# UWQuickstep/quickstep

Measured on AMD Instinct MI355X. Metric: probe+aggregate rows/s at TPC-H SF100 (Q1,Q3), higher is better.
Workload: dtype i32 keys / f64 sums

## Files before the change

### quickstep_amd/csrc/aggregate.hip

```cpp

#include "agg_common.hpp"
#include "agg_translate.hpp"
#include "agg_hash_update.hpp"
#include "agg_factored.hpp"
#include "agg_shapes.hpp"
#include "agg_family.hpp"
#include "agg_pieces.hpp"
#include "agg_jit.hpp"
#include "comm.hpp"
#include "partition.hpp"
#include "scan.hpp"

#include <atomic>
#include <cstdlib>
#include <map>
#include <mutex>
#include <shared_mutex>
#include <vector>

namespace qsx {

struct ColKinds {
  int kind[QSX_MAX_AGGS + 1];
};

__global__ __launch_bounds__(kABlock) void fill_identity_kernel(unsigned long long *__restrict__ states, long long col_stride,
                                                               long long col_words, int num_cols, ColKinds kinds) {
  for (int col = 0; col < num_cols; ++col) {
    if (kinds.kind[col] < kAccMinI64) continue;
    const unsigned long long identity = static_cast<unsigned long long>(acc_identity(kinds.kind[col]));
    unsigned long long *p = states + static_cast<long long>(col) * col_stride;
    for (long long i = static_cast<long long>(blockIdx.x) * kABlock + threadIdx.x; i < col_words;
         i += static_cast<long long>(gridDim.x) * kABlock) {
      p[i] = identity;
    }
  }
}

__global__ __launch_bounds__(kABlock) void merge_hash_kernel(const unsigned long long *__restrict__ image,
                                                            unsigned long long src_cap, int num_cols,
                                                            ColKinds kinds, HashTableView g) {
  const unsigned long long *src_keys = image;
  const unsigned long long *src_states = image + (src_cap + 1);
  for (unsigned long long i = static_cast<unsigned long long>(blockIdx.x) * kABlock + threadIdx.x;
       i <= src_cap; i += static_cast<unsigned long long>(gridDim.x) * kABlock) {
    const unsigned long long cnt = src_states[i];
    if (cnt == 0) continue;
    const unsigned long long code = i == src_cap ? kEmptyCode : src_keys[i];
    if (i != src_cap && code == kEmptyCode) continue;
    const unsigned long long gs = global_find_or_insert(g, code);
    if (gs == ~0ull) continue;
    for (int col = 0; col < num_cols; ++col) {
      global_add(g, col, gs, src_states[static_cast<unsigned long long>(col) * (src_cap + 1) + i], kinds.kind[col]);
    }
  }
}

__global__ __launch_bounds__(kABlock) void merge_dense_kernel(const unsigned long long *__restrict__ image,
                                                             unsigned long long *__restrict__ dst,
                                                             long long exist_words, long long num_entries,
                                                             int num_cols, ColKinds kinds) {
  const long long total = exist_words + static_cast<long long>(num_cols) * num_entries;
  for (long long i = static_cast<long long>(blockIdx.x) * kABlock + threadIdx.x; i < total;
       i += static_cast<long long>(gridDim.x) * kABlock) {
    const unsigned long long v = image[i];
    if (i < exist_words) {
      if (v != 0) atomicOr(&dst[i], v);
    } else {
      const int kind = kinds.kind[static_cast<int>((i - exist_words) / num_entries)];
      if (v == static_cast<unsigned long long>(acc_identity(kind))) continue;
      global_accumulate(&dst[i], v, kind);
    }
  }
}

__global__ __launch_bounds__(kABlock) void init_log_kernel(unsigned long long *__restrict__ log, int stride,
                                                          unsigned long long count, const unsigned int *__restrict__ count_dev,
                                                          unsigned int log_cap, ColKinds kinds) {
  if (count_dev != nullptr) count = *count_dev < log_cap ? *count_dev : log_cap;
  const unsigned long long words = count * stride;
  for (unsigned long long i = static_cast<unsigned long long>(blockIdx.x) * kABlock + threadIdx.x; i < words;
       i += static_cast<unsigned long long>(gridDim.x) * kABlock) {
    const int w = static_cast<int>(i % stride);
    log[i] = w == 0 ? kEmptyCode : static_cast<unsigned long long>(acc_identity(kinds.kind[w - 1]));
  }
}

__global__ __launch_bounds__(kABlock) void drain_log_kernel(const unsigned long long *__restrict__ records, unsigned int count,
                                                           int stride, int num_cols, ColKinds kinds, HashTableView g) {
  for (unsigned int r = blockIdx.x * kABlock + threadIdx.x; r < count; r += gridDim.x * kABlock) {
    const unsigned long long *rec = records + static_cast<unsigned long long>(r) * stride;
    const unsigned long long gs = global_find_or_insert(g, rec[0]);
    if (gs == ~0ull) continue;
    for (int col = 0; col < num_cols; ++col) global_add(g, col, gs, rec[1 + col], kinds.kind[col]);
  }
}

__global__ void publish_control_kernel(const unsigned long long *__restrict__ control, unsigned long long *host_slot,
                                       unsigned long long seq) {
  if (threadIdx.x != 0) return;
  __hip_atomic_store(&host_slot[0], control[0], __ATOMIC_RELAXED, __HIP_MEMORY_SCOPE_SYSTEM);
  __hip_atomic_store(&host_slot[1], control[3], __ATOMIC_RELAXED, __HIP_MEMORY_SCOPE_SYSTEM);
  __hip_atomic_store(&host_slot[2], control[1], __ATOMIC_RELAXED, __HIP_MEMORY_SCOPE_SYSTEM);
  __hip_atomic_store(&host_slot[3], seq, __ATOMIC_RELEASE, __HIP_MEMORY_SCOPE_SYSTEM);
}


__device__ __forceinline__ double avg_quotient(double s, double c) {
  const double q = s / c;
  if (!isfinite(q) || fabs(q) >= 2.2250738585072014e-308) return q;
  double best = q, best_r = fabs(fma(-q, c, s));
  const double around[2] = {nextafter(q, -INFINITY), nextafter(q, INFINITY)};
  for (const double x : around) {
    const double r = fabs(fma(-x, c, s));
    if (r < best_r || (r == best_r && (__double_as_longlong(x) & 1) == 0)) {
      best = x;
      best_r = r;
    }
  }
  return best;
}

__device__ __forceinline__ void write_values(const FinalizeDesc &f, const unsigned long long *states,
                                             unsigned long long col_stride, unsigned long long idx,
                                             int count_col, bool empty_group, long long out_row) {
  const long long cnt = count_col >= 0 ? static_cast<long long>(states[static_cast<unsigned long long>(count_col) * col_stride + idx]) : 0;
  for (int a = 0; a < f.num_aggs; ++a) {
    bool is_null = false;
    const bool has_nn = f.nn_col[a] >= 0;
    const long long seen = has_nn ? static_cast<long long>(states[static_cast<unsigned long long>(f.nn_col[a]) * col_stride + idx]) : cnt;
    if (f.fn[a] == QSX_AGG_COUNT_STAR) {
      static_cast<long long *>(f.out_vals[a])[out_row] = cnt;
    } else if (f.fn[a] == QSX_AGG_COUNT) {
      static_cast<long long *>(f.out_vals[a])[out_row] = seen;
    } else {
      const unsigned long long raw = states[static_cast<unsigned long long>(f.sum_col[a]) * col_stride + idx];
      if (f.fn[a] == QSX_AGG_SUM) {
        is_null = empty_group || (has_nn && seen == 0);
        static_cast<unsigned long long *>(f.out_vals[a])[out_row] = is_null ? 0ull : raw;
      } else if (f.fn[a] == QSX_AGG_MIN || f.fn[a] == QSX_AGG_MAX) {
        is_null = empty_group || (has_nn ? seen == 0 : (count_col >= 0 && cnt == 0));
        const long long word = static_cast<long long>(raw);
        switch (f.val_type[a]) {
          case QSX_INT: static_cast<int32_t *>(f.out_vals[a])[out_row] = is_null ? 0 : static_cast<int32_t>(word); break;
          case QSX_LONG: static_cast<long long *>(f.out_vals[a])[out_row] = is_null ? 0 : word; break;
          case QSX_FLOAT:
            static_cast<float *>(f.out_vals[a])[out_row] = is_null ? 0.0f : static_cast<float>(__longlong_as_double(ordered_from_bits(word)));
            break;
          default:
            static_cast<double *>(f.out_vals[a])[out_row] = is_null ? 0.0 : __longlong_as_double(ordered_from_bits(word));
            break;
        }
      } else {
        const double sum = f.is_int[a] ? static_cast<double>(static_cast<long long>(raw))
                                       : __longlong_as_double(static_cast<long long>(raw));
        is_null = seen == 0;
        static_cast<double *>(f.out_vals[a])[out_row] = is_null ? 0.0 : avg_quotient(sum, static_cast<double>(seen));
      }
// ... 739 lines not shown
}
static int dir_plane_sums(const DevConfig &dev) { return dev.num_sums - 2 * dev.wide_words; }
static size_t dir_lds_bytes(int tile_bytes, int temps_bytes, int num_sums, int gids, int nbuf) {
  return static_cast<size_t>(nbuf) * tile_bytes + temps_bytes + static_cast<size_t>(gids + kWave) * (8 * static_cast<size_t>(num_sums) + 4) + 16;
}

struct DenseLdsGeometry {
  int entries;
  int rep_shift;
  int ranges;
};
static DenseLdsGeometry dense_lds_geometry(long long num_entries, int num_sums, size_t tile_and_temps_bytes, bool allow_families) {
  const char *e = getenv("QSX_AGG_DENSE_LDS");
  constexpr long long kMaxRanges = 8;
  const size_t per_entry = 8 * static_cast<size_t>(num_sums) + 4;
  const size_t fixed = tile_and_temps_bytes + kWave * per_entry + 16;
  if ((e != nullptr && e[0] == '0') || num_entries <= 0 || fixed + 64 * per_entry > 160 * 1024) return DenseLdsGeometry{0, 0, 1};
  const long long capacity = static_cast<long long>((160 * 1024 - fixed) / per_entry / 64 * 64);
  if (num_entries > capacity * kMaxRanges) return DenseLdsGeometry{0, 0, 1};
  if (num_entries > capacity) {
    if (!allow_families) return DenseLdsGeometry{0, 0, 1};
    const long long ranges = (num_entries + capacity - 1) / capacity;
    const long long per = ((num_entries + ranges - 1) / ranges + 63) / 64 * 64;
    return DenseLdsGeometry{static_cast<int>(per), 0, static_cast<int>(ranges)};
  }
  int rep_shift = 0;
  while (rep_shift < 6 && (num_entries << (rep_shift + 1)) <= 2048) ++rep_shift;
  return DenseLdsGeometry{static_cast<int>(num_entries), rep_shift, 1};
}
static int dense_lds_grid(int64_t n, int ranges) {
  int grid = dir_grid(n * ranges) / ranges * ranges;
  return grid < ranges ? ranges : grid;
}

template <typename Shape>
static int launch_shape_dir(const void *const *cols, int num_columns, int64_t n, const HashTableView &g, const DirView &d, int gids,
                            int nbuf, hipStream_t stream, const long long *block_run) {
  constexpr Translated T = Shape::translated(kDirBlock);
  static_assert(T.status == QSX_OK, "plan shape does not translate");
  constexpr size_t kMaxLds = 160 * 1024;
  const size_t lds = dir_lds_bytes(T.dev.tile_bytes, 0, T.num_sums - 2 * T.dev.wide_words, gids, nbuf);
  if (lds > kMaxLds) return QSX_ERR_CAPACITY;
  static PerDeviceOnce attribute_set;
  {
    const int rc = once_per_device(attribute_set, [] {
      return hipFuncSetAttribute(reinterpret_cast<const void *>(&agg_dir_shape_kernel<Shape>),
                                 hipFuncAttributeMaxDynamicSharedMemorySize, static_cast<int>(kMaxLds));
    });
    if (rc != QSX_OK) return rc;
  }
  if (block_run != nullptr) {
    static PerDeviceOnce runs_attribute_set;
    const int rc = once_per_device(runs_attribute_set, [] {
      return hipFuncSetAttribute(reinterpret_cast<const void *>(&agg_dir_shape_runs_kernel<Shape>),
                                 hipFuncAttributeMaxDynamicSharedMemorySize, static_cast<int>(kMaxLds));
    });
    if (rc != QSX_OK) return rc;
    hipLaunchKernelGGL((agg_dir_shape_runs_kernel<Shape>), dim3(dir_grid(n)), dim3(kDirBlock), lds, stream, n, g, d, gids, nbuf, block_run);
    return QSX_OK;
  }
  ColumnPointers cp;
  for (int i = 0; i < QSX_MAX_COLUMNS; ++i) cp.p[i] = i < num_columns ? cols[i] : nullptr;
  if (nbuf == 2 && dir_rows_per_thread() == 2) {
    constexpr Translated W = Shape::translated(2 * kDirBlock);
    const size_t wide_lds = dir_lds_bytes(W.dev.tile_bytes, 0, W.num_sums - 2 * W.dev.wide_words, gids, 1);
    if (wide_lds <= kMaxLds) {
      static PerDeviceOnce wide_attribute_set;
      const int rc = once_per_device(wide_attribute_set, [] {
        return hipFuncSetAttribute(reinterpret_cast<const void *>(&agg_dir_shape_wide_kernel<Shape>),
                                   hipFuncAttributeMaxDynamicSharedMemorySize, static_cast<int>(kMaxLds));
      });
      if (rc != QSX_OK) return rc;
      hipLaunchKernelGGL((agg_dir_shape_wide_kernel<Shape>), dim3(dir_grid(n)), dim3(kDirBlock), wide_lds, stream, cp, n, g, d, gids);
      return QSX_OK;
    }
  }
  hipLaunchKernelGGL((agg_dir_shape_kernel<Shape>), dim3(dir_grid(n)), dim3(kDirBlock), lds, stream, cp, n, g, d, gids, nbuf);
  return QSX_OK;
}

static int launch_dir_build(DevConfig dc, unsigned key_columns, int64_t n, const uint64_t *filter, DirView d, int gids,
                            unsigned call, hipStream_t stream, const long long *block_run) {
  const char *e = getenv("QSX_AGG_DIR_SAMPLE_ROWS");
  const int64_t sample_rows = e != nullptr && atoll(e) > 0 ? atoll(e) : (4 << 20);
  const int64_t stride = std::max<int64_t>(1, std::min<int64_t>(64, n / sample_rows));
  d.sample_stride = static_cast<int>(stride);
  d.sample_phase = static_cast<int>(call % stride);
  QSX_HIP_TRY(hipMemsetAsync(d.bounds, 0, sizeof(unsigned long long) * 2 * QSX_MAX_KEYS, stream));
  plan_tile(dc, key_columns, kDirBlock, filter != nullptr);
  dc.temps_bytes = 0;
  constexpr size_t kMaxLds = 160 * 1024;
  const size_t slot_bytes = dc.wide_words != 0 ? 8 * (1 + static_cast<size_t>(kMaxKeyWords)) : 8;
  int slots = static_cast<int>(next_pow2(static_cast<uint64_t>(gids) * 2));
  int nbuf = 2;
  while (slots > 1024 && static_cast<size_t>(nbuf) * dc.tile_bytes + slot_bytes * static_cast<size_t>(slots) + 16 > kMaxLds) slots >>= 1;
  const size_t lds = static_cast<size_t>(nbuf) * dc.tile_bytes + slot_bytes * static_cast<size_t>(slots) + 16;
  if (lds > kMaxLds) return QSX_ERR_CAPACITY;
  static PerDeviceOnce attribute_set;
  {
    const int rc = once_per_device(attribute_set, [] {
      hipError_t err = hipFuncSetAttribute(reinterpret_cast<const void *>(&agg_dir_build_kernel<false>),
                                           hipFuncAttributeMaxDynamicSharedMemorySize, static_cast<int>(kMaxLds));
      if (err == hipSuccess) {
        err = hipFuncSetAttribute(reinterpret_cast<const void *>(&agg_dir_build_kernel<true>), hipFuncAttributeMaxDynamicSharedMemorySize,
                                  static_cast<int>(kMaxLds));
      }
      return err;
    });
    if (rc != QSX_OK) return rc;
  }
  const int64_t sampled_tiles = ((n + kDirBlock - 1) / kDirBlock - d.sample_phase + stride - 1) / stride;
  const int grid = static_cast<int>(std::max<int64_t>(1, std::min<int64_t>(sampled_tiles, kCUs)));
  for (int step = 0; step < 2; ++step) {
    d.build_step = step;
    const size_t step_lds = step == 0 ? static_cast<size_t>(nbuf) * dc.tile_bytes + 16 : lds;
    if (block_run != nullptr) {
      hipLaunchKernelGGL(agg_dir_build_kernel<true>, dim3(grid), dim3(kDirBlock), step_lds, stream, dc, n, filter, d, slots, nbuf, block_run);
    } else {
      hipLaunchKernelGGL(agg_dir_build_kernel<false>, dim3(grid), dim3(kDirBlock), step_lds, stream, dc, n, filter, d, slots, nbuf, block_run);
    }
  }
  return QSX_OK;
}

template <int NS>
static int launch_dir(DevConfig dc, unsigned used_columns, int64_t n, const uint64_t *filter, const HashTableView &g, const DirView &d,
                      int gids, int nbuf, hipStream_t stream, const long long *block_run) {
  plan_tile(dc, used_columns, kDirBlock, filter != nullptr);
  plan_interpreter(dc, kDirBlock);
  constexpr size_t kMaxLds = 160 * 1024;
  const size_t lds = dir_lds_bytes(dc.tile_bytes, dc.temps_bytes, dir_plane_sums(dc), gids, nbuf);
  if (lds > kMaxLds) return QSX_ERR_CAPACITY;
  static PerDeviceOnce attribute_set;
  {
    const int rc = once_per_device(attribute_set, [] {
      hipError_t err = hipFuncSetAttribute(reinterpret_cast<const void *>(&agg_dir_update_kernel<NS, false>),
                                           hipFuncAttributeMaxDynamicSharedMemorySize, static_cast<int>(kMaxLds));
      if (err == hipSuccess) {
        err = hipFuncSetAttribute(reinterpret_cast<const void *>(&agg_dir_update_kernel<NS, true>),
                                  hipFuncAttributeMaxDynamicSharedMemorySize, static_cast<int>(kMaxLds));
      }
      return err;
    });
    if (rc != QSX_OK) return rc;
  }
  if (block_run != nullptr) {
    hipLaunchKernelGGL((agg_dir_update_kernel<NS, true>), dim3(dir_grid(n)), dim3(kDirBlock), lds, stream, dc, n, filter, g, d, gids, nbuf, block_run);
  } else {
    hipLaunchKernelGGL((agg_dir_update_kernel<NS, false>), dim3(dir_grid(n)), dim3(kDirBlock), lds, stream, dc, n, filter, g, d, gids, nbuf, block_run);
  }
  return QSX_OK;
}

template <typename Shape, int V>
static int launch_shape_v(const void *const *cols, int num_columns, int64_t n, const HashTableView &g, int S,
                          int ranges, const long long *pieces, hipStream_t stream, bool runs) {
  constexpr int TR = kABlock * V;
  constexpr Translated T = Shape::translated(TR);
  static_assert(T.status == QSX_OK, "plan shape does not translate");
  constexpr int NS = T.num_sums;
  const AggTuning &tune = agg_tuning();
  const int nbuf = tune.buffers == 0 ? 1 : tune.buffers;
  size_t lds = 0;
  const int rep_shift = choose_replication(NS, S, static_cast<size_t>(nbuf) * T.dev.tile_bytes, tune, &lds);
  constexpr size_t kMaxLds = 160 * 1024;
  if (lds > kMaxLds) return QSX_ERR_CAPACITY;
  static PerDeviceOnce attribute_set;
  {
    const int rc = once_per_device(attribute_set, [] {
      return hipFuncSetAttribute(reinterpret_cast<const void *>(&agg_hash_shape_kernel<Shape, V>),
                                 hipFuncAttributeMaxDynamicSharedMemorySize, static_cast<int>(kMaxLds));
    });
    if (rc != QSX_OK) return rc;
  }
  int per_cu = static_cast<int>(kMaxLds / ((lds + 1023) / 1024 * 1024));
  if (per_cu > tune.max_blocks_per_cu) per_cu = tune.max_blocks_per_cu;
  if (per_cu < 1) per_cu = 1;
  const int64_t num_tiles = (n + TR - 1) / TR;
  const int64_t max_grid = static_cast<int64_t>(kCUs) * per_cu;
  int grid = static_cast<int>(num_tiles * ranges < max_grid ? num_tiles * ranges : max_grid);
  grid = grid / ranges * ranges;
  if (grid < ranges) grid = ranges;
  ColumnPointers cp;
  for (int i = 0; i < QSX_MAX_COLUMNS; ++i) cp.p[i] = i < num_columns ? cols[i] : nullptr;
  if (getenv("QSX_DEBUG_LAUNCH") != nullptr) {
    std::fprintf(stderr, "[qsx] shape launch grid=%d lds=%zu S=%d rep_shift=%d nbuf=%d ranges=%d tile_bytes=%d n=%lld\n", grid, lds, S,
                 rep_shift, nbuf, ranges, T.dev.tile_bytes, static_cast<long long>(n));
  }
#define QSX_LAUNCH_FIXED(S_, REP_, RANGES_, REG_)                                                                                  \
  do {                                                                                                                             \
    static PerDeviceOnce fixed_attribute_set;                                                                                      \
    const int attr_rc = once_per_device(fixed_attribute_set, [] {                                                                  \
      return hipFuncSetAttribute(reinterpret_cast<const void *>(&agg_hash_shape_fixed_kernel<Shape, V, S_, REP_, RANGES_, REG_>),  \
                                 hipFuncAttributeMaxDynamicSharedMemorySize, static_cast<int>(kMaxLds));                          \
    });                                                                                                                            \
    if (attr_rc != QSX_OK) return attr_rc;                                                                                         \
    hipLaunchKernelGGL((agg_hash_shape_fixed_kernel<Shape, V, S_, REP_, RANGES_, REG_>), dim3(grid), dim3(kABlock), lds, stream,   \
                       cp, n, g, pieces);                                                                                          \
    return QSX_OK;                                                                                                                 \
  } while (0)
  if (runs && nbuf == 1 && S == 16 && rep_shift == 4 && ranges == 1) {
    static PerDeviceOnce fixed_runs_attribute_set;
    const int rc = once_per_device(fixed_runs_attribute_set, [] {
      hipError_t err = hipFuncSetAttribute(reinterpret_cast<const void *>(&agg_hash_shape_fixed_runs_kernel<Shape, V, 16, 4, 1, true>),
                                           hipFuncAttributeMaxDynamicSharedMemorySize, static_cast<int>(kMaxLds));
      if (err == hipSuccess) {
        err = hipFuncSetAttribute(reinterpret_cast<const void *>(&agg_hash_shape_fixed_runs_kernel<Shape, V, 16, 4, 1, false>),
                                  hipFuncAttributeMaxDynamicSharedMemorySize, static_cast<int>(kMaxLds));
      }
      return err;
    });
    if (rc != QSX_OK) return rc;
    if (reg_groups_enabled()) {
      hipLaunchKernelGGL((agg_hash_shape_fixed_runs_kernel<Shape, V, 16, 4, 1, true>), dim3(grid), dim3(kABlock), lds, stream, n, g, pieces);
    } else {
      hipLaunchKernelGGL((agg_hash_shape_fixed_runs_kernel<Shape, V, 16, 4, 1, false>), dim3(grid), dim3(kABlock), lds, stream, n, g, pieces);
    }
    return QSX_OK;
  }
  if (runs) {
    static PerDeviceOnce runs_attribute_set;
    const int rc = once_per_device(runs_attribute_set, [] {
      return hipFuncSetAttribute(reinterpret_cast<const void *>(&agg_hash_shape_runs_kernel<Shape, V>),
                                 hipFuncAttributeMaxDynamicSharedMemorySize, static_cast<int>(kMaxLds));
    });
    if (rc != QSX_OK) return rc;
    hipLaunchKernelGGL((agg_hash_shape_runs_kernel<Shape, V>), dim3(grid), dim3(kABlock), lds, stream, n, g, S, rep_shift, nbuf, ranges, pieces);
    return QSX_OK;
  }
  if (nbuf == 1 && S == 16 && rep_shift == 4 && ranges == 1 && pieces == nullptr) {
    if (reg_groups_enabled()) QSX_LAUNCH_FIXED(16, 4, 1, true);
    QSX_LAUNCH_FIXED(16, 4, 1, false);
  }
  if (nbuf == 1 && S == 1024 && rep_shift == 0 && ranges == 32 && pieces != nullptr) QSX_LAUNCH_FIXED(1024, 0, 32, false);
#undef QSX_LAUNCH_FIXED
  hipLaunchKernelGGL((agg_hash_shape_kernel<Shape, V>), dim3(grid), dim3(kABlock), lds, stream, cp, n, g, S, rep_shift, nbuf,
                     ranges, pieces);
  return QSX_OK;
}

template <typename Shape>
static int launch_shape(const void *const *cols, int num_columns, int64_t n, const HashTableView &g, int S,
                        int ranges, const long long *pieces, hipStream_t stream, bool runs) {
  if (agg_tuning().shape_rows_per_thread == 4) return launch_shape_v<Shape, 4>(cols, num_columns, n, g, S, ranges, pieces, stream, runs);
  return launch_shape_v<Shape, 2>(cols, num_columns, n, g, S, ranges, pieces, stream, runs);
}

int qsx::shape_launch_geometry(int NS, int S, int tile_bytes, ShapeGeometry *out) {
  const AggTuning &tune = agg_tuning();
  out->nbuf = tune.buffers == 0 ? 1 : tune.buffers;
  out->rep_shift = choose_replication(NS, S, static_cast<size_t>(out->nbuf) * tile_bytes, tune, &out->lds);
  constexpr size_t kMaxLds = 160 * 1024;
  if (out->lds > kMaxLds) return QSX_ERR_CAPACITY;
  int per_cu = static_cast<int>(kMaxLds / ((out->lds + 1023) / 1024 * 1024));
  if (per_cu > tune.max_blocks_per_cu) per_cu = tune.max_blocks_per_cu;
  out->per_cu = per_cu < 1 ? 1 : per_cu;
  return QSX_OK;
}

static const FamilyEntry *find_family(const qsx_agg_config_t &c, const DevConfig &d, int num_sums, int *num_columns, int *cols) {
  if (getenv("QSX_AGG_NO_SPECIALIZE") != nullptr && atoi(getenv("QSX_AGG_NO_SPECIALIZE")) != 0) return nullptr;
  if (getenv("QSX_AGG_FAMILY") != nullptr && atoi(getenv("QSX_AGG_FAMILY")) == 0) return nullptr;
  if (c.strategy != QSX_AGG_COMPACT_KEY && c.strategy != QSX_AGG_GENERIC) return nullptr;
  if (d.num_keys < 1 || d.num_keys > 2 || d.wide_words != 0 || d.num_instrs != 0 || d.num_null_cols != 0) return nullptr;
  for (int p = 0; p < d.num_pred; ++p) {
    const int col = d.pred[p].column, type = d.column_type[col];
    if (d.code_width[col] != 0 || c.column_nullable[col] != 0) return nullptr;
    if (type != QSX_INT && type != QSX_LONG && type != QSX_FLOAT && type != QSX_DOUBLE && type != QSX_DATE) return nullptr;
  }
  if (num_sums < 1 || num_sums > kFamilyMaxSums) return nullptr;
  int kt[2] = {0, 0}, n = 0;
  for (int k = 0; k < d.num_keys; ++k) {
    const int col = d.key_column[k], type = d.column_type[col];
    if (d.code_width[col] != 0 || c.column_nullable[col] != 0) return nullptr;
    if (!((type == QSX_CHAR && d.column_width[col] == 1) || type == QSX_INT || type == QSX_LONG)) return nullptr;
    kt[k] = d.column_width[col];
    cols[n++] = col;
  }
  for (int j = 0; j < num_sums; ++j) {
    const DevSum &sum = d.sums[j];
    if (sum.kind != kAccSumF64 || sum.count_valid != 0 || sum.null_mask != 0 || sum.is_int != 0 || sum.arg.kind != QSX_OPD_COLUMN) return nullptr;
    const int col = sum.arg.index;
    if (d.column_type[col] != QSX_DOUBLE || d.code_width[col] != 0 || c.column_nullable[col] != 0) return nullptr;
    cols[n++] = col;
  }
  const FamilyEntry *e = find_family_entry(kt[0], kt[1], num_sums);
  if (e != nullptr) *num_columns = n;
  return e;
}

static bool family_serves_runs(const qsx_agg_state *st) { return st->family != nullptr && !st->dense && st->dev.num_pred == 0 && st->dir_gids == 0; }
static std::atomic<long long> g_family_launches{0};
extern "C" long long qsx_debug_agg_family_launches(void) { return g_family_launches.load(std::memory_order_relaxed); }

static const ShapeEntry *find_shape(const qsx_agg_config_t &c) {
  static const ShapeEntry table[] = {
      {"tpch_q1", ShapeTpchQ1::config(), &launch_shape<ShapeTpchQ1>, &launch_shape_dir<ShapeTpchQ1>},
      {"two_int_keys_sum_count_avg", ShapeTwoIntKeysSumCountAvg::config(), &launch_shape<ShapeTwoIntKeysSumCountAvg>,
       &launch_shape_dir<ShapeTwoIntKeysSumCountAvg>},
  };
  if (getenv("QSX_AGG_NO_SPECIALIZE") != nullptr && atoi(getenv("QSX_AGG_NO_SPECIALIZE")) != 0) return nullptr;
  for (const ShapeEntry &e : table) {
    if (same_plan(e.config, c)) return &e;
  }
  return nullptr;
}

static long long jit_min_rows() {
  const char *e = getenv("QSX_AGG_JIT_MIN_ROWS");
  if (e != nullptr) return atoll(e);
  return jit_compiles_out_of_process() ? 256ll * 1024 : 2048ll * 1024;
}

static JitGeometry jit_geometry_for(const qsx_agg_state *st, int tile_bytes, int slots, int num_ranges, size_t *lds) {
  const int NS = st->num_sums;
  JitGeometry g{};
  if (st->dense) {
    g = JitGeometry{8, 0, 1, 1};
    *lds = static_cast<size_t>(tile_bytes) + sizeof(unsigned long long) * (8 + static_cast<size_t>(NS + 1) * (8 + kWave));
    return g;
  }
  const AggTuning &tune = agg_tuning();
  g.S = slots;
  g.ranges = num_ranges;
  g.nbuf = tune.buffers;
  int decoded_columns = 0;
  for (int col = 0; col < st->dev.num_columns; ++col) {
    decoded_columns += st->dev.code_width[col] != 0 && ((st->used_columns >> col) & 1u) != 0 ? 1 : 0;
  }
  const size_t dict_bytes = static_cast<size_t>(decoded_columns) * kDictLdsEntries * 8;
  if (tune.buffers == 0) {
    size_t with_two = 0;
    choose_replication(NS, g.S, 2 * static_cast<size_t>(tile_bytes) + dict_bytes, tune, &with_two);
    g.nbuf = (with_two + 1023) / 1024 * 1024 * 3 <= 160 * 1024 ? 2 : 1;
  }
  g.rep_shift = choose_replication(NS, g.S, static_cast<size_t>(g.nbuf) * tile_bytes + dict_bytes, tune, lds);
  g.reg_groups = reg_groups_enabled() && g.ranges == 1 ? reg_groups_for(g.S, NS) : 0;
  const int by_lds = static_cast<int>(160 * 1024 / ((*lds + 1023) / 1024 * 1024));
  g.waves_per_eu = by_lds >= 5 && g.reg_groups == 0 && tune.jit_waves_per_eu != 0 ? tune.jit_waves_per_eu : 0;
  return g;
}

static const JitKernel *state_jit_kernel(qsx_agg_state *st, bool has_filter, bool partitioned, int slots, int num_ranges, int64_t n,
                                         int *variant, bool directory = false, bool runs = false) {
  const long long seen = st->rows_seen.fetch_add(n) + n;
  const int v = (has_filter ? 1 : 0) + (runs && directory ? 8 : (runs ? 6 : (directory ? 4 : (partitioned ? 2 : 0))));
  *variant = v;
  std::lock_guard<std::mutex> lock(st->jit_mutex);
  if (st->jit_tried[v]) return st->jit[v];
  if (st->jit_request[v] == nullptr) {
    const long long min_rows = jit_min_rows();
    if (seen < min_rows) return nullptr;
    if (getenv("QSX_AGG_NO_SPECIALIZE") != nullptr && atoi(getenv("QSX_AGG_NO_SPECIALIZE")) != 0) {
      st->jit_tried[v] = true;
      return nullptr;
    }
    DevConfig dev = st->dev;
    DenseLdsGeometry dense_lds{0, 0, 1};
    if (st->dense) {
      plan_tile(dev, st->used_columns, kDirBlock, has_filter);
      dense_lds = dense_lds_geometry(st->config.num_entries, st->num_sums, static_cast<size_t>(dev.tile_bytes), st->dense_families.load() == 1);
    }
    plan_tile(dev, st->used_columns, directory || dense_lds.entries != 0 ? kDirBlock : kABlock * jit_rows_per_thread(), has_filter,
              !directory && dense_lds.entries == 0);
    st->jit_tile_bytes[v] = dev.tile_bytes;
    if (dense_lds.entries != 0) {
      const int copies = dense_lds.entries << dense_lds.rep_shift;
      int nbuf = 2;
      size_t lds = dir_lds_bytes(dev.tile_bytes, 0, st->num_sums, copies, nbuf);
      if (lds > 160 * 1024) lds = dir_lds_bytes(dev.tile_bytes, 0, st->num_sums, copies, nbuf = 1);
      st->jit_geometry[v] = JitGeometry{dense_lds.entries, dense_lds.rep_shift, nbuf, dense_lds.ranges, copies, runs ? 1 : 0};
      st->jit_lds[v] = lds;
      if (dir_rows_per_thread() == 2 && nbuf == 2 && !runs) {
        for (int rows_per_thread = 4; rows_per_thread >= 2; rows_per_thread >>= 1) {
          DevConfig wide = dev;
          plan_tile(wide, st->used_columns, rows_per_thread * kDirBlock, has_filter);
          const size_t wide_lds = dir_lds_bytes(wide.tile_bytes, 0, st->num_sums, copies, 1);
          if (wide_lds > 160 * 1024) continue;
          dev = wide;
          st->jit_tile_bytes[v] = dev.tile_bytes;
          st->jit_geometry[v].nbuf = 1;
          st->jit_geometry[v].dir_rows = rows_per_thread;
          st->jit_lds[v] = wide_lds;
// ... 2240 lines not shown
```

Before: 181.4 billion.

## Add register-resident streaming aggregation kernel for small-cardinality char-key plans

Adds a new streaming kernel for TPC-H Q1-like plans with 1-byte char keys and double sums. Each wave holds up to four group accumulators in registers and adopts new keys through a ballot/readlane loop. It loads two rows per thread with nontemporal vector loads and double-buffers tiles. Overflow groups spill to a small LDS table and then to the global hash table. The aim is to replace the replicated-LDS hash update with mostly register accumulation and wider loads, at the cost of a specialised path with more register pressure that is gated by an env var and a minimum row count.

```diff
diff --git a/quickstep_amd/csrc/agg_stream.hip b/quickstep_amd/csrc/agg_stream.hip
--- /dev/null
+++ b/quickstep_amd/csrc/agg_stream.hip
@@ -0,0 +1,287 @@
+#include "agg_stream.hpp"
+
+#include <algorithm>
+#include <cstdio>
+#include <cstdlib>
+
+namespace qsx {
+namespace {
+
+typedef double f64x2 __attribute__((ext_vector_type(2)));
+
+template <typename V>
+__device__ __forceinline__ V stream_load_nt(const char *p) {
+  return __builtin_nontemporal_load((const __attribute__((address_space(1))) V *)reinterpret_cast<uintptr_t>(p));
+}
+
+constexpr bool stream_value_column(const DevConfig &d, unsigned used, int col) {
+  if (col >= d.num_columns || ((used >> col) & 1u) == 0) return false;
+  for (int k = 0; k < d.num_keys; ++k) {
+    if (d.key_column[k] == col) return false;
+  }
+  return true;
+}
+
+template <int U>
+struct StreamRows {
+  f64x2 v[QSX_MAX_COLUMNS][U];
+  uint16_t k[QSX_MAX_KEYS][U];
+};
+
+template <int NS, typename Code>
+struct StreamState {
+  double acc[kStreamGroups][NS];
+  unsigned int cnt[kStreamGroups];
+  Code key[kStreamGroups];
+  int held;
+};
+
+template <int U, int BLOCK, bool kFull>
+__device__ __forceinline__ void stream_load(const DevConfig &c, unsigned used, const StreamColumns &cols, int64_t n, int64_t tile,
+                                            StreamRows<U> &r) {
+#pragma unroll
+  for (int u = 0; u < U; ++u) {
+    const int64_t row = (tile * U + u) * (2 * BLOCK) + 2 * static_cast<int64_t>(threadIdx.x);
+#pragma unroll
+    for (int k = 0; k < QSX_MAX_KEYS; ++k) {
+      if (k < c.num_keys) {
+        const char *p = static_cast<const char *>(cols.p[c.key_column[k]]) + row;
+        uint16_t x = 0;
+        if (kFull || row + 1 < n) {
+          x = stream_load_nt<uint16_t>(p);
+        } else if (row < n) {
+          x = stream_load_nt<uint8_t>(p);
+        }
+        r.k[k][u] = x;
+      }
+    }
+#pragma unroll
+    for (int col = 0; col < QSX_MAX_COLUMNS; ++col) {
+      if (stream_value_column(c, used, col)) {
+        const char *p = static_cast<const char *>(cols.p[col]) + row * 8;
+        f64x2 x = {0.0, 0.0};
+        if (kFull || row + 1 < n) {
+          x = stream_load_nt<f64x2>(p);
+        } else if (row < n) {
+          x.x = stream_load_nt<double>(p);
+        }
+        r.v[col][u] = x;
+      }
+    }
+  }
+}
+
+__device__ __forceinline__ uint32_t stream_read_lane(uint32_t v, int lane) {
+  return static_cast<uint32_t>(__builtin_amdgcn_readlane(static_cast<int>(v), lane));
+}
+__device__ __forceinline__ unsigned long long stream_bits(double v) { return static_cast<unsigned long long>(__double_as_longlong(v)); }
+
+template <int NS>
+__device__ __forceinline__ void stream_table_add(unsigned long long *l_keys, unsigned long long *l_acc, const HashTableView &g,
+                                                 unsigned long long code, unsigned long long rows, const double (&sum)[NS]) {
+  const int s = lds_find_or_insert(l_keys, kStreamSlots, code);
+  if (s >= 0) {
+    lds_add(&l_acc[s], rows, kAccSumI64);
+#pragma unroll
+    for (int j = 0; j < NS; ++j) lds_add(&l_acc[(j + 1) * kStreamSlots + s], stream_bits(sum[j]), kAccSumF64);
+    return;
+  }
+  const unsigned long long gs = global_find_or_insert(g, code);
+  if (gs != ~0ull) {
+    global_add(g, 0, gs, rows, kAccSumI64);
+#pragma unroll
+    for (int j = 0; j < NS; ++j) global_add(g, j + 1, gs, stream_bits(sum[j]), kAccSumF64);
+  }
+  __builtin_amdgcn_s_waitcnt(0x0F70);
+}
+
+template <int NS, typename Code>
+__device__ __forceinline__ void stream_accumulate(StreamState<NS, Code> &st, int e, bool m, const double (&val)[NS]) {
+#pragma unroll
+  for (int j = 0; j < NS; ++j) st.acc[e][j] += m ? val[j] : 0.0;
+  st.cnt[e] += m ? 1u : 0u;
+}
+
+template <int U, int BLOCK, bool kFull, int NS, typename Code>
+__device__ __forceinline__ void stream_compute(const DevConfig &c, int64_t n, int64_t tile, const StreamRows<U> &r,
+                                               StreamState<NS, Code> &st, unsigned long long *l_keys, unsigned long long *l_acc,
+                                               const HashTableView &g) {
+  static_assert(U == 1, "put #pragma unroll back on the step loop");
+  for (int u = 0; u < U; ++u) {
+    const int64_t row = (tile * U + u) * (2 * BLOCK) + 2 * static_cast<int64_t>(threadIdx.x);
+    Code code[2];
+    bool live[2], unmatched[2];
+    double val[2][NS];
+#pragma unroll
+    for (int i = 0; i < 2; ++i) {
+      live[i] = kFull || row + i < n;
+      code[i] = 0;
+#pragma unroll
+      for (int k = 0; k < QSX_MAX_KEYS; ++k) {
+        if (k < c.num_keys) {
+          code[i] |= ((static_cast<uint32_t>(r.k[k][u]) >> (8 * i)) & 0xFFu) << c.key_shift[k];
+        }
+      }
+      double temps[QSX_MAX_TEMPS] = {};
+      auto operand = [&](const DevOperand &o) __attribute__((always_inline)) {
+        return o.kind == QSX_OPD_CONST ? c.consts[o.index] : (o.kind == QSX_OPD_TEMP ? temps[o.index] : r.v[o.index][u][i]);
+      };
+#pragma unroll
+      for (int t = 0; t < QSX_MAX_INSTRS; ++t) {
+        if (t < c.num_instrs) {
+          const double a = operand(c.instrs[t].a), b = operand(c.instrs[t].b);
+          const int op = c.instrs[t].op;
+          temps[c.instrs[t].dst] = op == QSX_EX_ADD ? a + b : (op == QSX_EX_SUB ? a - b : (op == QSX_EX_MUL ? a * b : a / b));
+        }
+      }
+#pragma unroll
+      for (int j = 0; j < NS; ++j) val[i][j] = operand(c.sums[j].arg);
+      bool any = false;
+#pragma unroll
+      for (int e = 0; e < kStreamGroups; ++e) {
+        const bool m = live[i] && e < st.held && code[i] == st.key[e];
+        stream_accumulate(st, e, m, val[i]);
+        any = any || m;
+      }
+      unmatched[i] = live[i] && !any;
+    }
+    while (true) {
+      const unsigned long long waiting = __ballot(unmatched[0] || unmatched[1]);
+      if (waiting == 0) break;
+      if (st.held == kStreamGroups) {
+#pragma unroll
+        for (int i = 0; i < 2; ++i) {
+          if (unmatched[i]) stream_table_add<NS>(l_keys, l_acc, g, code[i], 1ull, val[i]);
+        }
+        break;
+      }
+      const Code adopted = stream_read_lane(unmatched[0] ? code[0] : code[1], __builtin_ctzll(waiting));
+#pragma unroll
+      for (int e = 0; e < kStreamGroups; ++e) {
+        if (e == st.held) {
+          st.key[e] = adopted;
+#pragma unroll
+          for (int i = 0; i < 2; ++i) stream_accumulate(st, e, unmatched[i] && code[i] == adopted, val[i]);
+        }
+      }
+      st.held += 1;
+#pragma unroll
+      for (int i = 0; i < 2; ++i) unmatched[i] = unmatched[i] && code[i] != adopted;
+    }
+  }
+}
+
+template <typename Shape, int U, int BLOCK>
+__global__ __launch_bounds__(BLOCK) void agg_stream_kernel(StreamColumns cols, int64_t n, HashTableView g) {
+  static constexpr Translated T = Shape::translated(2 * BLOCK * U);
+  static_assert(stream_serves(T), "the stream kernel does not take this plan shape");
+  constexpr int NS = T.num_sums;
+  constexpr unsigned kUsed = T.used_columns;
+  constexpr int64_t TR = 2 * BLOCK * U;
+  using Code = uint32_t;
+  __shared__ unsigned long long l_keys[kStreamSlots];
+  __shared__ unsigned long long l_acc[(NS + 1) * kStreamSlots];
+  for (int i = threadIdx.x; i < kStreamSlots; i += BLOCK) l_keys[i] = kEmptyCode;
+  for (int i = threadIdx.x; i < (NS + 1) * kStreamSlots; i += BLOCK) l_acc[i] = 0ull;
+  __syncthreads();
+
+  StreamState<NS, Code> st;
+#pragma unroll
+  for (int e = 0; e < kStreamGroups; ++e) {
+    st.cnt[e] = 0u;
+    st.key[e] = 0;
+#pragma unroll
+    for (int j = 0; j < NS; ++j) st.acc[e][j] = 0.0;
+  }
+  st.held = 0;
+
+  const int64_t num_full = n / TR, stride = gridDim.x;
+  int64_t t = blockIdx.x;
+  if (t < num_full) {
+    StreamRows<U> a, b;
+    stream_load<U, BLOCK, true>(T.dev, kUsed, cols, n, t, a);
+    while (t + stride < num_full) {
+      stream_load<U, BLOCK, true>(T.dev, kUsed, cols, n, t + stride, b);
+      __builtin_amdgcn_sched_barrier(0);
+      stream_compute<U, BLOCK, true>(T.dev, n, t, a, st, l_keys, l_acc, g);
+      t += stride;
+      stream_load<U, BLOCK, true>(T.dev, kUsed, cols, n, t + stride < num_full ? t + stride : t, a);
+      __builtin_amdgcn_sched_barrier(0);
+      stream_compute<U, BLOCK, true>(T.dev, n, t, b, st, l_keys, l_acc, g);
+      t += stride;
+    }
+    if (t < num_full) stream_compute<U, BLOCK, true>(T.dev, n, t, a, st, l_keys, l_acc, g);
+  }
+  if (num_full * TR < n && static_cast<int64_t>(blockIdx.x) == num_full % stride) {
+    StreamRows<U> a;
+    stream_load<U, BLOCK, false>(T.dev, kUsed, cols, n, num_full, a);
+    stream_compute<U, BLOCK, false>(T.dev, n, num_full, a, st, l_keys, l_acc, g);
+  }
+
+#pragma unroll
+  for (int e = 0; e < kStreamGroups; ++e) {
+    const unsigned long long rows = wave_reduce_add(static_cast<unsigned long long>(st.cnt[e]));
+    double sum[NS];
+#pragma unroll
+    for (int j = 0; j < NS; ++j) sum[j] = wave_reduce_add(st.acc[e][j]);
+    if (lane_id() == 0 && e < st.held && rows != 0) {
+      stream_table_add<NS>(l_keys, l_acc, g, static_cast<unsigned long long>(st.key[e]), rows, sum);
+    }
+  }
+  __syncthreads();
+  for (int sl = threadIdx.x; sl < kStreamSlots; sl += BLOCK) {
+    const unsigned long long code = l_keys[sl], rows = l_acc[sl];
+    if (code == kEmptyCode || rows == 0) continue;
+    const unsigned long long gs = global_find_or_insert(g, code);
+    if (gs == ~0ull) continue;
+    global_add(g, 0, gs, rows, kAccSumI64);
+#pragma unroll
+    for (int j = 0; j < NS; ++j) global_add(g, j + 1, gs, l_acc[(j + 1) * kStreamSlots + sl], kAccSumF64);
+  }
+}
+
+constexpr int kStreamU = 1;
+constexpr int kStreamBlock = 256;
+
+}
+
+bool agg_stream_enabled() {
+  const char *e = getenv("QSX_AGG_STREAM");
+  return e == nullptr || atoi(e) != 0;
+}
+
+static int64_t stream_min_rows() {
+  const char *e = getenv("QSX_AGG_STREAM_MIN_ROWS");
+  return e != nullptr ? atoll(e) : 2000000;
+}
+
+template <typename Shape>
+bool AggStream<Shape>::takes(const void *const *cols, int num_columns, int64_t n) {
+  static constexpr Translated T = Shape::translated(kABlock);
+  if (n <= 0 || n < stream_min_rows()) return false;
+  for (int col = 0; col < T.dev.num_columns; ++col) {
+    if (((T.used_columns >> col) & 1u) == 0) continue;
+    if (col >= num_columns || cols[col] == nullptr) return false;
+    const uintptr_t bytes = stream_value_column(T.dev, T.used_columns, col) ? 16 : 2;
+    if (reinterpret_cast<uintptr_t>(cols[col]) % bytes != 0) return false;
+  }
+  return true;
+}
+
+template <typename Shape>
+int AggStream<Shape>::launch(const void *const *cols, int num_columns, int64_t n, const HashTableView &g, hipStream_t stream) {
+  if (n <= 0) return QSX_ERR_INVALID_ARGUMENT;
+  StreamColumns cp;
+  for (int i = 0; i < QSX_MAX_COLUMNS; ++i) cp.p[i] = i < num_columns ? cols[i] : nullptr;
+  constexpr int64_t tile_rows = 2ll * kStreamBlock * kStreamU;
+  const int grid = static_cast<int>(std::min<int64_t>((n + tile_rows - 1) / tile_rows, kCUs));
+  if (getenv("QSX_DEBUG_LAUNCH") != nullptr) {
+    std::fprintf(stderr, "[qsx] stream launch grid=%d block=%d n=%lld\n", grid, kStreamBlock, static_cast<long long>(n));
+  }
+  hipLaunchKernelGGL((agg_stream_kernel<Shape, kStreamU, kStreamBlock>), dim3(grid), dim3(kStreamBlock), 0, stream, cp, n, g);
+  return QSX_OK;
+}
+
+template struct AggStream<ShapeTpchQ1>;
+
+}
diff --git a/quickstep_amd/csrc/agg_stream.hpp b/quickstep_amd/csrc/agg_stream.hpp
--- /dev/null
+++ b/quickstep_amd/csrc/agg_stream.hpp
@@ -0,0 +1,54 @@
+#ifndef QSX_CSRC_AGG_STREAM_HPP_
+#define QSX_CSRC_AGG_STREAM_HPP_
+
+#include "agg_shapes.hpp"
+
+namespace qsx {
+
+constexpr int kStreamGroups = 4;
+constexpr int kStreamSlots = 16;
+
+constexpr bool stream_serves(const Translated &t) {
+  const DevConfig &d = t.dev;
+  if (t.status != QSX_OK || t.dense || d.wide_words != 0 || d.num_pred != 0 || d.num_null_cols != 0) return false;
+  if (d.num_keys < 1 || t.num_sums < 1 || t.num_sums > 6) return false;
+  bool is_key[QSX_MAX_COLUMNS] = {};
+  for (int k = 0; k < d.num_keys; ++k) {
+    const int col = d.key_column[k], type = d.column_type[col];
+    if (type != QSX_CHAR || d.key_width[k] != 1) return false;
+    is_key[col] = true;
+  }
+  for (int col = 0; col < d.num_columns; ++col) {
+    if (d.code_width[col] != 0) return false;
+    if (((t.used_columns >> col) & 1u) && !is_key[col] && d.column_type[col] != QSX_DOUBLE) return false;
+  }
+  auto double_operand = [&](const DevOperand &o) {
+    return o.kind == QSX_OPD_CONST || o.kind == QSX_OPD_TEMP || (o.kind == QSX_OPD_COLUMN && d.column_type[o.index] == QSX_DOUBLE);
+  };
+  for (int i = 0; i < d.num_instrs; ++i) {
+    if (d.instrs[i].op < QSX_EX_ADD || d.instrs[i].op >= QSX_EX_IADD) return false;
+    if (!double_operand(d.instrs[i].a) || !double_operand(d.instrs[i].b)) return false;
+  }
+  for (int j = 0; j < t.num_sums; ++j) {
+    const DevSum &s = d.sums[j];
+    if (s.kind != kAccSumF64 || s.is_int != 0 || s.count_valid != 0 || s.null_mask != 0) return false;
+    if (s.arg.kind == QSX_OPD_CONST || !double_operand(s.arg)) return false;
+  }
+  return true;
+}
+
+struct StreamColumns {
+  const void *p[QSX_MAX_COLUMNS];
+};
+
+template <typename Shape>
+struct AggStream {
+  static bool takes(const void *const *cols, int num_columns, int64_t n);
+  static int launch(const void *const *cols, int num_columns, int64_t n, const HashTableView &g, hipStream_t stream);
+};
+
+bool agg_stream_enabled();
+
+}
+
+#endif
diff --git a/quickstep_amd/csrc/aggregate.hip b/quickstep_amd/csrc/aggregate.hip
--- a/quickstep_amd/csrc/aggregate.hip
+++ b/quickstep_amd/csrc/aggregate.hip
@@ -4,6 +4,7 @@
 #include "agg_hash_update.hpp"
 #include "agg_factored.hpp"
 #include "agg_shapes.hpp"
+#include "agg_stream.hpp"
 #include "agg_family.hpp"
 #include "agg_pieces.hpp"
 #include "agg_jit.hpp"
@@ -1049,6 +1050,9 @@
   return QSX_OK;
 }
 
+static std::atomic<long long> g_stream_launches{0};
+extern "C" long long qsx_debug_agg_stream_launches(void) { return g_stream_launches.load(std::memory_order_relaxed); }
+
 template <typename Shape, int V>
 static int launch_shape_v(const void *const *cols, int num_columns, int64_t n, const HashTableView &g, int S,
                           int ranges, const long long *pieces, hipStream_t stream, bool runs) {
@@ -1126,6 +1130,13 @@
     return QSX_OK;
   }
   if (nbuf == 1 && S == 16 && rep_shift == 4 && ranges == 1 && pieces == nullptr) {
+    if constexpr (stream_serves(T)) {
+      if (!reg_groups_enabled() && agg_stream_enabled() && AggStream<Shape>::takes(cols, num_columns, n)) {
+        const int stream_rc = AggStream<Shape>::launch(cols, num_columns, n, g, stream);
+        if (stream_rc == QSX_OK) g_stream_launches.fetch_add(1, std::memory_order_relaxed);
+        return stream_rc;
+      }
+    }
     if (reg_groups_enabled()) QSX_LAUNCH_FIXED(16, 4, 1, true);
     QSX_LAUNCH_FIXED(16, 4, 1, false);
   }
```

New measurement: 187.6 billion, median of 6. 3.4% higher.
